# stevesuyao/KinectDepthMapEnhancement

Hardware: AMD Instinct MI355X
Metric: Mpixels/sec joint-bilateral filtered (640x480 & 1080p); % HBM roofline (higher is better)
Workload: dtype f32; 1 GPU; JointBilateralFilter::Process (K0 pre-smooth 5/30/30 + K1) on 64 x 640x480 synthetic RGB-D frames (64 per GPU), window 11 (radius 5), sigma_s 3 px, sigma_r 7.65/255, sigma_d 20 mm; frames_per_gpu=64, width=640, height=480, window=11, kernel_variant=auto (w11-pk2-16x16-false-v4)

## Files before the change

### kinectdepthmapenhancement_amd/csrc/jbf_fast.hip

```cpp
#include "kde_internal.h"
#include "kde_device_math.h"

#include <type_traits>

namespace kde {
namespace {

constexpr uint32_t kMagic = 0x4B000000u;
constexpr uint32_t kOff = 1u << 18;
constexpr uint32_t kInvalidBias = 0xFF000000u;
constexpr float kBiasF = 8388608.0f + 262144.0f;
constexpr uint32_t kNegHBits = 0xCB7C0000u;
constexpr double kScaleLog2 = 24.0;

struct FastArgs {
    const float* depth;
    const uint8_t* guide;
    float* out;
    int width, height, n;
    int tiles_x, tiles_y;
    FastDiv24 div_tiles, div_tx;
    float kc;
    float sd;
    float t_skip;
    float t2_skip;
    int cd_skip;
    int vec4;
    KDE_STAGE(float* stage_avg; unsigned* stage_counters; int stage_force;)
    const float* tab_dev;
    __attribute__((aligned(8))) float tab[882];
};

__device__ __forceinline__ uint32_t dot4(uint32_t a, uint32_t b, uint32_t c)
{
    return __builtin_amdgcn_udot4(a, b, c, false);
}


template <int WIN, int PX, int BX, int BY, bool CACHE, bool CSKIP>
__global__ __launch_bounds__(BX* BY) void jbf_fast_kernel(const FastArgs a)
{
    constexpr int R = WIN / 2;
    constexpr int NT = BX * BY;
    constexpr int TW = BX * PX, TH = BY;
    constexpr int LW = TW + 2 * R, LH = TH + 2 * R;
    constexpr int P = LW;
    constexpr int SEG = PX + 2 * R;
    __shared__ float s_d[LH * P];
    __shared__ uint32_t s_c[LH * P];
    __shared__ uint32_t s_n[LH * P];

    const unsigned nblk = gridDim.x;
    const unsigned lin = blockIdx.x;
    const unsigned per = nblk / 8, rem = nblk % 8;
    const unsigned xcd = lin % 8, slot = lin / 8;
    const unsigned id = xcd * per + (xcd < rem ? xcd : rem) + slot;
    const unsigned tiles = (unsigned)a.tiles_x * a.tiles_y;
    const unsigned frame_i = fastdiv24(id, a.div_tiles);
    const unsigned tile = id - frame_i * tiles;
    const int tyi = (int)fastdiv24(tile, a.div_tx), txi = tile - tyi * a.tiles_x;
    const int x0 = txi * TW, y0 = tyi * TH;

    const size_t frame = (size_t)frame_i * a.width * a.height;
    const float* __restrict__ depth = a.depth + frame;
    const uint8_t* __restrict__ guide = a.guide + frame * 3;
    const int tid = threadIdx.x;

    for (int i = tid; i < LW * LH; i += NT) {
        const int ly = i / LW, lx = i - ly * LW;
        const int gx = x0 + lx - R, gy = y0 + ly - R;
        float d = 0.0f;
        uint32_t c = 0;
        if (gx >= 0 && gx < a.width && gy >= 0 && gy < a.height) {
            const size_t q = (size_t)gy * a.width + gx;
            d = depth[q];
            const uint8_t* p = guide + q * 3;
            c = (uint32_t)p[0] | ((uint32_t)p[1] << 8) | ((uint32_t)p[2] << 16);
        }
        const bool valid = d > 50.0f;
        s_d[ly * P + lx] = valid ? d : 0.0f;
        s_c[ly * P + lx] = c;
        s_n[ly * P + lx] = valid ? (kMagic + kOff) - dot4(c, c, 0) : kInvalidBias;
    }
    __syncthreads();

    const int tx = tid % BX, ty = tid / BX;
    const int xb = x0 + tx * PX, y = y0 + ty;
    if (xb >= a.width || y >= a.height) return;

    uint32_t cc[PX];
    float cA[PX], skipA[PX];
    uint32_t thrU[PX];
#pragma unroll
    for (int k = 0; k < PX; k++) {
        cc[k] = s_c[(ty + R) * P + tx * PX + R + k];
        const uint32_t na = dot4(cc[k], cc[k], 0);
        cA[k] = -a.kc * (kBiasF + (float)na);
        skipA[k] = __builtin_fmaf(kBiasF + (float)na, a.kc, cA[k]);
        thrU[k] = CSKIP ? (kMagic + kOff) + na - (uint32_t)a.cd_skip : 0;
    }

    float arg[CACHE ? WIN * WIN * PX : 1];
    float wsum[PX], wgt[PX];
#pragma unroll
    for (int k = 0; k < PX; k++) wsum[k] = wgt[k] = 0.0f;

    auto arg1_of = [&](uint32_t cq, uint32_t nq, int k, float ls) -> float {
        const uint32_t u = (dot4(cq, cc[k], 0) << 1) + nq;
        float a1 = __builtin_fmaf(__uint_as_float(u), a.kc, cA[k]);
        if (CSKIP) a1 = (u <= thrU[k]) ? skipA[k] : a1;
        return a1 + ls;
    };

    auto pass1_row = [&](int i) {
        float dr[SEG];
        uint32_t cr[SEG], nr[SEG];
        const int rb = (ty + i) * P + tx * PX;
#pragma unroll
        for (int q = 0; q < SEG; q++) {
            dr[q] = s_d[rb + q];
            cr[q] = s_c[rb + q];
            nr[q] = s_n[rb + q];
        }
#pragma unroll
        for (int j = 0; j < WIN; j++) {
            const float ls = a.tab[i * WIN + j];
#pragma unroll
            for (int k = 0; k < PX; k++) {
                const float a1 = arg1_of(cr[j + k], nr[j + k], k, ls);
                if (CACHE) arg[(i * WIN + j) * PX + k] = a1;
                const float f = __builtin_amdgcn_exp2f(a1);
                wsum[k] = __builtin_fmaf(dr[j + k], f, wsum[k]);
                wgt[k] += f;
            }
        }
    };
    if (CACHE) {
#pragma unroll
        for (int i = 0; i < WIN; i++) pass1_row(i);
    } else {
#pragma unroll 1
        for (int i = 0; i < WIN; i++) pass1_row(i);
    }

    float c2[PX], num[PX], den[PX];
#pragma unroll
    for (int k = 0; k < PX; k++) {
        c2[k] = wsum[k] / wgt[k];
        num[k] = den[k] = 0.0f;
    }

    auto pass2_row = [&](int i) {
        float dr[SEG];
        uint32_t cr[SEG], nr[SEG];
        const int rb = (ty + i) * P + tx * PX;
#pragma unroll
        for (int q = 0; q < SEG; q++) {
            dr[q] = s_d[rb + q];
            if (!CACHE) {
                cr[q] = s_c[rb + q];
                nr[q] = s_n[rb + q];
            }
        }
#pragma unroll
        for (int j = 0; j < WIN; j++) {
            const float ls = CACHE ? 0.0f : a.tab[i * WIN + j];
#pragma unroll
            for (int k = 0; k < PX; k++) {
                const float a1 = CACHE ? arg[(i * WIN + j) * PX + k] : arg1_of(cr[j + k], nr[j + k], k, ls);
                const float t = (dr[j + k] - c2[k]) * a.sd;
                float a2 = __builtin_fmaf(-t, t, a1);
                a2 = (__builtin_fabsf(t) >= a.t_skip) ? a1 : a2;
                const float f = __builtin_amdgcn_exp2f(a2);
                num[k] = __builtin_fmaf(dr[j + k], f, num[k]);
                den[k] += f;
            }
        }
    };
    if (CACHE) {
#pragma unroll
        for (int i = 0; i < WIN; i++) pass2_row(i);
    } else {
#pragma unroll 1
        for (int i = 0; i < WIN; i++) pass2_row(i);
    }

    float* __restrict__ o = a.out + frame + (size_t)y * a.width + xb;
#pragma unroll
    for (int k = 0; k < PX; k++) {
        float r = 0.0f;
        if (wgt[k] > 0.0f) r = (den[k] == 0.0f) ? 0.0f : num[k] / den[k];
        if (xb + k < a.width) o[k] = r;
        KDE_STAGE(if (a.stage_avg && xb + k < a.width) a.stage_avg[frame + (size_t)y * a.width + xb + k] = c2[k];)
    }
}


typedef float f2 __attribute__((ext_vector_type(2)));
typedef uint32_t u2 __attribute__((ext_vector_type(2)));

__device__ __forceinline__ f2 pk_fma(f2 a, f2 b, f2 c) { return __builtin_elementwise_fma(a, b, c); }
__device__ __forceinline__ f2 bcast(float v) { return f2{v, v}; }
__device__ __forceinline__ f2 pk_add_clamp(f2 a, f2 b)
{
    f2 r;
    asm("v_pk_add_f32 %0, %1, %2 clamp" : "=v"(r) : "v"(a), "v"(b));
    return r;
}
__device__ __forceinline__ f2 pk_mul_clamp(f2 a, f2 b)
{
    f2 r;
    asm("v_pk_mul_f32 %0, %1, %2 clamp" : "=v"(r) : "v"(a), "v"(b));
    return r;
}

typedef unsigned short us2 __attribute__((ext_vector_type(2)));
__device__ __forceinline__ uint32_t pk_min_u16(uint32_t a, uint32_t b)
{
    return __builtin_bit_cast(uint32_t, __builtin_elementwise_min(__builtin_bit_cast(us2, a), __builtin_bit_cast(us2, b)));
}
__device__ __forceinline__ uint32_t pk_max_u16(uint32_t a, uint32_t b)
{
    return __builtin_bit_cast(uint32_t, __builtin_elementwise_max(__builtin_bit_cast(us2, a), __builtin_bit_cast(us2, b)));
}
template <int CTRL, int ROWS = 0xf>
__device__ __forceinline__ uint32_t dpp_mov(uint32_t v)
{
    return (uint32_t)__builtin_amdgcn_update_dpp((int)v, (int)v, CTRL, ROWS, 0xf, false);
}
template <class Op>
__device__ __forceinline__ uint32_t wave_reduce(uint32_t v, Op op)
{
    v = op(v, dpp_mov<0xb1>(v));
    v = op(v, dpp_mov<0x4e>(v));
    v = op(v, dpp_mov<0x124>(v));
    v = op(v, dpp_mov<0x128>(v));
    v = op(v, dpp_mov<0x142, 0xa>(v));
    v = op(v, dpp_mov<0x143, 0xc>(v));
    return (uint32_t)__builtin_amdgcn_readlane((int)v, 63);
}

constexpr int pk_min_waves(int win, int np, bool cache, bool cskip, bool elide_on)
{
    if (win >= 23) return 3;
    if (win == 5 && np == 1 && cache) return 5;
    if (np == 1 && !cskip && elide_on && !cache && win >= 9 && win <= 15) return win == 9 ? 8 : win == 11 ? 6 : 5;
    return 1;
}

template <int WIN, int NP, int BX, int BY, bool CACHE, bool CSKIP, bool VL, bool ELIDE_ON = true, int WTX = BX>
__global__ __launch_bounds__(BX* BY) __attribute__((amdgpu_waves_per_eu(pk_min_waves(WIN, NP, CACHE, CSKIP, ELIDE_ON))))
void jbf_pk_kernel(const FastArgs a)
{
    constexpr int CR = CACHE ? WIN : 0;
    constexpr int R = WIN / 2;
    constexpr int PX = 2 * NP;
    constexpr int NT = BX * BY;
    constexpr int WTY = 64 / WTX, WAVES_X = BX / WTX;
    static_assert(NT % 64 == 0 && 64 % WTX == 0 && BX % WTX == 0 && BY % WTY == 0, "whole wavefronts, each a WTX x WTY block of threads");
    constexpr int TW = BX * PX, TH = BY;
    constexpr int LH = TH + 2 * R;
    constexpr int S1 = 0;
    constexpr int RA = !VL ? R : ((R + 3) / 4 * 4);
    constexpr int SH = VL ? ((RA - R) & 1) : 0;
    constexpr bool ALIGNED = ((RA - R + SH) % 2) == 0;
    constexpr int G = (RA + TW + R + 3) / 4;
    constexpr int P = VL ? (SH + 4 * G + 1) / 2 * 2 : (TW + 2 * R);
    constexpr int SEGP = NP + R;
    constexpr int HALF = (WIN - 1) / 2;
    static_assert(RA >= R && P % 2 == 0 && (!VL || ((RA + S1) % 4 == 0 && TW % 4 == 0 && (SH != 0 || P % 4 == 0))), "tile geometry");
    __shared__ __attribute__((aligned(16))) float s_d[LH * P];
    __shared__ __attribute__((aligned(16))) uint32_t s_c[LH * P];
    __shared__ __attribute__((aligned(16))) float s_n[LH * P];

    const unsigned nblk = gridDim.x;
    const unsigned lin = blockIdx.x;
    const unsigned per = nblk / 8, rem = nblk % 8;
    const unsigned xcd = lin % 8, slot = lin / 8;
    const unsigned id = xcd * per + (xcd < rem ? xcd : rem) + slot;
    const unsigned tiles = (unsigned)a.tiles_x * a.tiles_y;
    const unsigned frame_i = fastdiv24(id, a.div_tiles);
    const unsigned tile = id - frame_i * tiles;
    const int tyi = (int)fastdiv24(tile, a.div_tx), txi = tile - tyi * a.tiles_x;
    const int x0 = txi * TW - S1, y0 = tyi * TH;
    const int o = x0 - RA;

    const size_t frame = (size_t)frame_i * a.width * a.height;
    const float* __restrict__ depth = a.depth + frame;
    const uint8_t* __restrict__ guide = a.guide + frame * 3;
    const int tid = threadIdx.x;

    constexpr bool ELIDE = WIN >= 9 && ELIDE_ON;

    if (!VL) {
        for (int i = tid; i < P * LH; i += NT) {
            const int ly = i / P, lx = i - ly * P;
            const int gx = o + lx, gy = y0 - R + ly;
            float d = 0.0f;
            uint32_t c = 0;
            const bool inside = gx >= 0 && gx < a.width && gy >= 0 && gy < a.height;
            if (inside) {
                const size_t q = (size_t)gy * a.width + gx;
                d = depth[q];
                const uint8_t* p = guide + q * 3;
                c = (uint32_t)p[0] | ((uint32_t)p[1] << 8) | ((uint32_t)p[2] << 16);
            }
            const bool valid = d > 50.0f;
            s_d[i] = valid ? d : 0.0f;
            s_c[i] = c;
            s_n[i] = __uint_as_float(dot4(c, c, kNegHBits));
        }
    }
    for (int g = tid; VL && g < G * LH; g += NT) {
        const int ly = g / G, gi = g - ly * G;
        const int gx = o + 4 * gi, gy = y0 - R + ly;
        float d[4] = {0.0f, 0.0f, 0.0f, 0.0f};
        uint32_t c[4] = {0u, 0u, 0u, 0u};
        if (gy >= 0 && gy < a.height) {
            const size_t q = (size_t)gy * a.width + gx;
            if (a.vec4 && gx >= 0 && gx + 3 < a.width) {
                const float4 dv = *reinterpret_cast<const float4*>(depth + q);
                const uint32_t* cp = reinterpret_cast<const uint32_t*>(guide + q * 3);
                const uint32_t w0 = cp[0], w1 = cp[1], w2 = cp[2];
                d[0] = dv.x; d[1] = dv.y; d[2] = dv.z; d[3] = dv.w;
                c[0] = w0 & 0xffffffu;
                c[1] = (w0 >> 24) | ((w1 & 0xffffu) << 8);
                c[2] = (w1 >> 16) | ((w2 & 0xffu) << 16);
                c[3] = w2 >> 8;
            } else {
#pragma unroll
                for (int k = 0; k < 4; k++) {
                    if (gx + k >= 0 && gx + k < a.width) {
                        d[k] = depth[q + k];
                        const uint8_t* p = guide + (q + k) * 3;
                        c[k] = (uint32_t)p[0] | ((uint32_t)p[1] << 8) | ((uint32_t)p[2] << 16);
                    }
                }
            }
        }
        float nn[4];
#pragma unroll
        for (int k = 0; k < 4; k++) {
            const bool valid = d[k] > 50.0f;
            d[k] = valid ? d[k] : 0.0f;
            nn[k] = __uint_as_float(dot4(c[k], c[k], kNegHBits));
        }
        const int li = ly * P + 4 * gi + SH;
        if constexpr (SH == 0) {
            *reinterpret_cast<float4*>(&s_d[li]) = make_float4(d[0], d[1], d[2], d[3]);
            *reinterpret_cast<uint4*>(&s_c[li]) = make_uint4(c[0], c[1], c[2], c[3]);
            *reinterpret_cast<float4*>(&s_n[li]) = make_float4(nn[0], nn[1], nn[2], nn[3]);
        } else {
#pragma unroll
            for (int k = 0; k < 4; k++) {
                s_d[li + k] = d[k];
                s_c[li + k] = c[k];
                s_n[li + k] = nn[k];
            }
        }
    }
    __syncthreads();

    const int wave = __builtin_amdgcn_readfirstlane(tid >> 6), lane = tid & 63;
    const int tx0 = WTX * (wave % WAVES_X), ty0 = WTY * (wave / WAVES_X);
    const int tx = tx0 + lane % WTX, ty = ty0 + lane / WTX;
    if (x0 + tx0 * PX >= a.width || y0 + ty0 >= a.height) return;

    bool tile_c = CSKIP, tile_d = true;
    if constexpr (ELIDE) {
        constexpr int RWP = (WTX * PX + 2 * R) / 2, RH = WTY + 2 * R;
        constexpr int NE = RWP * RH;
        const int sxw = SH + RA - R + tx0 * PX;
        const int gx0 = x0 + tx0 * PX - R, gy0 = y0 + ty0 - R;
        uint32_t dmin = 0xffffffffu, dmax = 0u;
        uint32_t brmin = 0x00ff00ffu, brmax = 0u, ggmin = 0x00ff00ffu, ggmax = 0u;
        auto scan = [&](auto masked_tag) {
            constexpr bool MASKED = decltype(masked_tag)::value;
            constexpr int QY = 64 / RWP, QP = 64 % RWP;
            int ry = lane / RWP, rp = lane - ry * RWP;
            int li = (ty0 + ry) * P + sxw + 2 * rp;
#pragma unroll
            for (int k = 0; k < (NE + 63) / 64; k++) {
                if (k > 0) {
                    const bool wrap = rp + QP >= RWP;
                    rp += wrap ? QP - RWP : QP;
                    ry += wrap ? QY + 1 : QY;
                    li += wrap ? (QY + 1) * P + 2 * (QP - RWP) : QY * P + 2 * QP;
                }
                if (64 * k + 63 < NE || lane + 64 * k < NE) {
                    const u2 d = *reinterpret_cast<const u2*>(&s_d[li]);
                    dmin = min(dmin, min(d.x - 1u, d.y - 1u));
                    dmax = max(dmax, max(d.x, d.y));
                    if constexpr (CSKIP) {
                        const u2 c = *reinterpret_cast<const u2*>(&s_c[li]);
                        uint32_t lo0 = c.x, lo1 = c.y, hi0 = c.x, hi1 = c.y;
                        if constexpr (MASKED) {
                            const bool iny = (unsigned)(gy0 + ry) < (unsigned)a.height;
                            const bool in0 = iny & ((unsigned)(gx0 + 2 * rp) < (unsigned)a.width);
                            const bool in1 = iny & ((unsigned)(gx0 + 2 * rp + 1) < (unsigned)a.width);
                            lo0 = in0 ? lo0 : 0x00ffffffu;
                            lo1 = in1 ? lo1 : 0x00ffffffu;
                            hi0 = in0 ? hi0 : 0u;
                            hi1 = in1 ? hi1 : 0u;
                        }
                        brmin = pk_min_u16(pk_min_u16(brmin, lo0 & 0x00ff00ffu), lo1 & 0x00ff00ffu);
                        brmax = pk_max_u16(pk_max_u16(brmax, hi0 & 0x00ff00ffu), hi1 & 0x00ff00ffu);
                        ggmin = pk_min_u16(ggmin, __builtin_amdgcn_perm(lo1, lo0, 0x0c050c01u));
                        ggmax = pk_max_u16(ggmax, __builtin_amdgcn_perm(hi1, hi0, 0x0c050c01u));
                    }
                }
            }
        };
        if (!CSKIP || (gx0 >= 0 && gx0 + 2 * RWP <= a.width && gy0 >= 0 && gy0 + RH <= a.height)) scan(std::false_type{});
        else scan(std::true_type{});
        const uint32_t w_dmin = wave_reduce(dmin, [](uint32_t p, uint32_t q) { return min(p, q); }) + 1u;
        const uint32_t w_dmax = wave_reduce(dmax, [](uint32_t p, uint32_t q) { return max(p, q); });
        if constexpr (CSKIP) {
            const uint32_t w_brmin = wave_reduce(brmin, pk_min_u16), w_brmax = wave_reduce(brmax, pk_max_u16);
            const uint32_t w_ggmin = wave_reduce(ggmin, pk_min_u16), w_ggmax = wave_reduce(ggmax, pk_max_u16);
            const int bmin = w_brmin & 0xffffu, bmax = w_brmax & 0xffffu, rmin = w_brmin >> 16, rmax = w_brmax >> 16;
            const int gmin = min(w_ggmin & 0xffffu, w_ggmin >> 16), gmax = max(w_ggmax & 0xffffu, w_ggmax >> 16);
            const int rb = bmax - bmin, rg = gmax - gmin, rr = rmax - rmin;
            if (bmax >= bmin) tile_c = rb * rb + rg * rg + rr * rr >= a.cd_skip;
        }
        if (w_dmax == 0u) {
            tile_d = false;
        } else {
            const float range = __uint_as_float(w_dmax) - __uint_as_float(w_dmin);
            const float slack = __uint_as_float(w_dmax) * (float)(WIN * WIN + 8) * 0x1p-24f;
            tile_d = !((range * 1.0001f + slack) * a.sd < a.t_skip);
        }
    }
    KDE_STAGE(if (a.stage_force) { tile_c = CSKIP; tile_d = true; })
    KDE_STAGE(if (a.stage_counters && lane == 0) {
        int body;
        if constexpr (!ELIDE) body = (CSKIP ? 1 : 0) + 2;
        else if constexpr (WIN >= 15) body = ((CSKIP && tile_c) || tile_d) ? (CSKIP ? 1 : 0) + 2 : 0;
        else body = ((CSKIP && tile_c) ? 1 : 0) + (tile_d ? 2 : 0);
        atomicAdd(&a.stage_counters[body], 1u);
    })

    const int xb = x0 + tx * PX, y = y0 + ty;
    if (xb >= a.width || y >= a.height) return;
    const int sx = SH + RA - R + tx * PX;

    uint32_t cc[PX];
    f2 negC[NP];
#pragma unroll
    for (int pp = 0; pp < NP; pp++) {
#pragma unroll
        for (int h = 0; h < 2; h++) {
            const int k = 2 * pp + h;
            cc[k] = s_c[(ty + R) * P + sx + R + k];
            const uint32_t na = dot4(cc[k], cc[k], 0);
            negC[pp][h] = -((float)kOff + (float)na);
        }
    }

    f2 kc2 = bcast(a.kc);
    asm volatile("" : "+v"(kc2));
    f2 arg[CR > 0 ? CR * WIN * NP : 1];
    f2 wsum[NP], wgt[NP];
#pragma unroll
    for (int pp = 0; pp < NP; pp++) wsum[pp] = wgt[pp] = bcast(0.0f);

    const f2 Tc = bcast((float)a.cd_skip);
    const f2 T2 = bcast(a.t2_skip);
    const f2 kBig = bcast(0x1p100f);

    auto unit_arg = [&](auto cs_tag, const u2* cp, const f2* np, int pp, int i, int u) -> f2 {
        constexpr bool CS = decltype(cs_tag)::value;
        uint32_t c0, c1;
        f2 hq;
        if (u <= HALF) {
            c0 = cp[pp + u].x; c1 = cp[pp + u].y; hq = np[pp + u];
        } else if (u < WIN - 1) {
            const int m = pp + (u - HALF);
            c0 = cp[m].y; c1 = cp[m].x; hq = __builtin_shufflevector(np[m], np[m], 1, 0);
        } else {
            c0 = cp[pp].y; c1 = cp[pp + HALF].x; hq = bcast(0.0f);
        }
        const f2 ab = f2{__uint_as_float(dot4(c0, cc[2 * pp], kMagic)), __uint_as_float(dot4(c1, cc[2 * pp + 1], kMagic))};
        f2 w;
        if (u == WIN - 1) {
            float w0 = __builtin_fmaf(ab.x, 2.0f, np[pp].y), w1 = __builtin_fmaf(ab.y, 2.0f, np[pp + HALF].x);
            asm("" : "+v"(w0));
            asm("" : "+v"(w1));
            w = f2{w0, w1};
        } else {
            w = pk_fma(ab, bcast(2.0f), hq);
        }
        const f2 ncd = w + negC[pp];
        f2 lsj;
        if constexpr (WIN > 21) {
            typedef const f2 __attribute__((address_space(4)))* cf2p;
            lsj = *(cf2p)(uintptr_t)(a.tab_dev + (i * WIN + u) * 2);
        } else {
            lsj = *reinterpret_cast<const f2*>(&a.tab[(i * WIN + u) * 2]);
        }
        if (CS) return pk_fma(ncd, pk_add_clamp(ncd, Tc) * kc2, lsj);
        return pk_fma(ncd, kc2, lsj);
    };
    auto unit_depth = [&](const f2* dp, int pp, int u) -> f2 {
        if (u <= HALF) return dp[pp + u];
        if (u < WIN - 1) return __builtin_shufflevector(dp[pp + (u - HALF)], dp[pp + (u - HALF)], 1, 0);
        return f2{dp[pp].y, dp[pp + HALF].x};
    };

    auto pass1_row = [&](auto cs_tag, auto keep_tag, int i) {
        constexpr bool KEEP = decltype(keep_tag)::value;
        f2 dp[SEGP], vp[SEGP];
        u2 cp[SEGP];
        f2 np[SEGP];
        const int rb = (ty + i) * P + sx;
#pragma unroll
        for (int m = 0; m < SEGP; m++) {
            dp[m] = ALIGNED ? *reinterpret_cast<const f2*>(&s_d[rb + 2 * m]) : f2{s_d[rb + 2 * m], s_d[rb + 2 * m + 1]};
            cp[m] = ALIGNED ? *reinterpret_cast<const u2*>(&s_c[rb + 2 * m]) : u2{s_c[rb + 2 * m], s_c[rb + 2 * m + 1]};
            np[m] = ALIGNED ? *reinterpret_cast<const f2*>(&s_n[rb + 2 * m]) : f2{s_n[rb + 2 * m], s_n[rb + 2 * m + 1]};
            vp[m] = pk_add_clamp(dp[m], dp[m]);
        }
#pragma unroll
        for (int pp = 0; pp < NP; pp++) {
#pragma unroll
            for (int u = 0; u < WIN; u++) {
                const f2 a1 = unit_arg(cs_tag, cp, np, pp, i, u);
                if constexpr (KEEP) arg[(i * NP + pp) * WIN + u] = a1;
                const f2 f = f2{__builtin_amdgcn_exp2f(a1.x), __builtin_amdgcn_exp2f(a1.y)};
                wsum[pp] = pk_fma(unit_depth(dp, pp, u), f, wsum[pp]);
                wgt[pp] = pk_fma(unit_depth(vp, pp, u), f, wgt[pp]);
            }
        }
    };
    f2 c2[NP], num[NP], den[NP];

    auto pass2_row = [&](auto cs_tag, auto ds_tag, auto keep_tag, int i) {
        constexpr bool DS = decltype(ds_tag)::value;
        constexpr bool KEEP = decltype(keep_tag)::value;
        f2 dp[SEGP], vp[SEGP];
        u2 cp[SEGP];
        f2 np[SEGP];
        const int rb = (ty + i) * P + sx;
#pragma unroll
        for (int m = 0; m < SEGP; m++) {
            dp[m] = ALIGNED ? *reinterpret_cast<const f2*>(&s_d[rb + 2 * m]) : f2{s_d[rb + 2 * m], s_d[rb + 2 * m + 1]};
            vp[m] = pk_add_clamp(dp[m], dp[m]);
            if constexpr (!KEEP) {
                cp[m] = ALIGNED ? *reinterpret_cast<const u2*>(&s_c[rb + 2 * m]) : u2{s_c[rb + 2 * m], s_c[rb + 2 * m + 1]};
                np[m] = ALIGNED ? *reinterpret_cast<const f2*>(&s_n[rb + 2 * m]) : f2{s_n[rb + 2 * m], s_n[rb + 2 * m + 1]};
            }
        }
#pragma unroll
        for (int pp = 0; pp < NP; pp++) {
#pragma unroll
            for (int u = 0; u < WIN; u++) {
                f2 a1;
                if constexpr (KEEP) a1 = arg[(i * NP + pp) * WIN + u];
                else a1 = unit_arg(cs_tag, cp, np, pp, i, u);
                const f2 dq = unit_depth(dp, pp, u);
                const f2 t = (dq - c2[pp]) * bcast(a.sd);
                f2 a2;
                if (DS) {
                    const f2 m = pk_mul_clamp(pk_fma(-t, t, T2), kBig);
                    a2 = pk_fma(-(t * m), t, a1);
                } else {
                    a2 = pk_fma(-t, t, a1);
                }
                const f2 f = f2{__builtin_amdgcn_exp2f(a2.x), __builtin_amdgcn_exp2f(a2.y)};
                num[pp] = pk_fma(dq, f, num[pp]);
                den[pp] = pk_fma(unit_depth(vp, pp, u), f, den[pp]);
            }
        }
    };
    auto run = [&](auto cs_tag, auto ds_tag) {
#pragma unroll
        for (int i = 0; i < CR; i++) pass1_row(cs_tag, std::true_type{}, i);
#pragma unroll 1
        for (int i = CR; i < WIN; i++) pass1_row(cs_tag, std::false_type{}, i);
#pragma unroll
        for (int pp = 0; pp < NP; pp++) {
            c2[pp] = wsum[pp] * f2{__builtin_amdgcn_rcpf(wgt[pp].x), __builtin_amdgcn_rcpf(wgt[pp].y)};
            num[pp] = den[pp] = bcast(0.0f);
        }
#pragma unroll
        for (int i = 0; i < CR; i++) pass2_row(cs_tag, ds_tag, std::true_type{}, i);
#pragma unroll 1
        for (int i = CR; i < WIN; i++) pass2_row(cs_tag, ds_tag, std::false_type{}, i);
    };
    using T_ = std::true_type;
    using F_ = std::false_type;
    if constexpr (!ELIDE) {
        run(std::integral_constant<bool, CSKIP>{}, T_{});
    } else if constexpr (WIN >= 15) {
        if ((CSKIP && tile_c) || tile_d) run(std::integral_constant<bool, CSKIP>{}, T_{});
        else run(F_{}, F_{});
    } else {
        if (!CSKIP || !tile_c) {
            if (tile_d) run(F_{}, T_{});
            else run(F_{}, F_{});
        } else {
            if (tile_d) run(T_{}, T_{});
            else run(T_{}, F_{});
        }
    }

    float* __restrict__ op = a.out + frame + (size_t)y * a.width + xb;
#pragma unroll
    for (int pp = 0; pp < NP; pp++) {
        float r0 = 0.0f, r1 = 0.0f;
        if (wgt[pp].x > 0.0f) r0 = (den[pp].x == 0.0f) ? 0.0f : num[pp].x * __builtin_amdgcn_rcpf(den[pp].x);
        if (wgt[pp].y > 0.0f) r1 = (den[pp].y == 0.0f) ? 0.0f : num[pp].y * __builtin_amdgcn_rcpf(den[pp].y);
        if (xb + 2 * pp >= 0 && xb + 2 * pp < a.width) op[2 * pp] = r0;
        if (xb + 2 * pp + 1 < a.width) op[2 * pp + 1] = r1;
        KDE_STAGE(if (a.stage_avg) {
            float* sp = a.stage_avg + frame + (size_t)y * a.width + xb;
            if (xb + 2 * pp >= 0 && xb + 2 * pp < a.width) sp[2 * pp] = c2[pp].x;
            if (xb + 2 * pp + 1 < a.width) sp[2 * pp + 1] = c2[pp].y;
        })
    }
}

template <int WIN, int NP, int BX, int BY, bool CACHE, bool VL, bool ELIDE_ON = true, int WTX = BX>
int launch_pk_variant(const JbfLaunch& l, const FastArgs& fa, bool cskip, hipStream_t s)
{
    FastArgs a = fa;
    a.tiles_x = ceil_div(l.width, BX * NP * 2);
    a.tiles_y = ceil_div(l.height, BY);
    const long long blocks = (long long)a.tiles_x * a.tiles_y * l.n;
    a.div_tiles = make_fastdiv24((uint32_t)(a.tiles_x * a.tiles_y), (uint64_t)blocks);
    a.div_tx = make_fastdiv24((uint32_t)a.tiles_x, (uint64_t)a.tiles_x * a.tiles_y);
    if (blocks > 0x7fffffffLL) return fail(KDE_ERR_INVALID, "jbf: batch too large for one launch");
    if (cskip)
        hipLaunchKernelGGL((jbf_pk_kernel<WIN, NP, BX, BY, CACHE, true, VL, ELIDE_ON, WTX>), dim3((unsigned)blocks), dim3(BX * BY), 0, s, a);
    else
        hipLaunchKernelGGL((jbf_pk_kernel<WIN, NP, BX, BY, CACHE, false, VL, ELIDE_ON, WTX>), dim3((unsigned)blocks), dim3(BX * BY), 0, s, a);
    KDE_HIP_TRY(hipGetLastError());
    return KDE_OK;
}

template <int WIN, int PX, int BX, int BY, bool CACHE>
int launch_variant(const JbfLaunch& l, const FastArgs& fa, bool cskip, hipStream_t s)
{
    FastArgs a = fa;
    a.tiles_x = ceil_div(l.width, BX * PX);
    a.tiles_y = ceil_div(l.height, BY);
    const long long blocks = (long long)a.tiles_x * a.tiles_y * l.n;
    a.div_tiles = make_fastdiv24((uint32_t)(a.tiles_x * a.tiles_y), (uint64_t)blocks);
    a.div_tx = make_fastdiv24((uint32_t)a.tiles_x, (uint64_t)a.tiles_x * a.tiles_y);
    if (blocks > 0x7fffffffLL) return fail(KDE_ERR_INVALID, "jbf: batch too large for one launch");
    if (cskip)
        hipLaunchKernelGGL((jbf_fast_kernel<WIN, PX, BX, BY, CACHE, true>), dim3((unsigned)blocks), dim3(BX * BY), 0, s, a);
    else
        hipLaunchKernelGGL((jbf_fast_kernel<WIN, PX, BX, BY, CACHE, false>), dim3((unsigned)blocks), dim3(BX * BY), 0, s, a);
    KDE_HIP_TRY(hipGetLastError());
    return KDE_OK;
}

struct Variant {
    const char* name;
    int window;
    bool packed;
    int (*launch)(const JbfLaunch&, const FastArgs&, bool, hipStream_t);
};

#define V(WIN, PX, BX, BY, CACHE) \
    {"w" #WIN "-sc" #PX "-" #BX "x" #BY "-" #CACHE, WIN, false, &launch_variant<WIN, PX, BX, BY, CACHE>}
#define K(WIN, NP, BX, BY, CACHE) \
    {"w" #WIN "-pk" #NP "-" #BX "x" #BY "-" #CACHE "-v4", WIN, true, &launch_pk_variant<WIN, NP, BX, BY, CACHE, true>}
#define KS(WIN, NP, BX, BY, CACHE) \
    {"w" #WIN "-pk" #NP "-" #BX "x" #BY "-" #CACHE "-v1", WIN, true, &launch_pk_variant<WIN, NP, BX, BY, CACHE, false>}
#define KN(WIN, NP, BX, BY, CACHE) \
    {"w" #WIN "-pk" #NP "-" #BX "x" #BY "-" #CACHE "-v4-noelide", WIN, true, &launch_pk_variant<WIN, NP, BX, BY, CACHE, true, false>}
#define KQ(WIN, NP, BX, BY, CACHE) \
    {"w" #WIN "-pk" #NP "-" #BX "x" #BY "-" #CACHE "-v4", WIN, true, &launch_pk_variant<WIN, NP, BX, BY, CACHE, true, true, 8>}
#define KR(WIN, NP, BX, BY, CACHE) \
    {"w" #WIN "-pk" #NP "-" #BX "x" #BY "-" #CACHE "-v4-rows", WIN, true, &launch_pk_variant<WIN, NP, BX, BY, CACHE, true>}
const Variant kVariants[] = {
    K(5, 1, 16, 16, true),  K(5, 1, 32, 8, true),   KS(5, 1, 16, 16, true),  K(5, 2, 32, 8, true),  K(5, 1, 32, 8, false),
    V(5, 2, 32, 8, true),   V(5, 1, 64, 4, true),
    K(7, 1, 16, 16, true),  K(7, 1, 32, 8, true),   KS(7, 1, 32, 8, true),  K(7, 1, 32, 8, false),  V(7, 1, 64, 4, true),
    KQ(11, 2, 16, 16, false), KR(11, 2, 16, 16, false), K(11, 2, 8, 32, false),
    KS(11, 2, 16, 16, false), KS(11, 1, 16, 16, false), K(11, 1, 16, 16, false), K(11, 1, 32, 8, false),
    KS(11, 1, 32, 8, false), KS(11, 2, 32, 8, false), V(11, 2, 16, 16, false), V(11, 1, 32, 8, false),
    KN(11, 2, 16, 16, false),
    K(19, 1, 16, 16, false), KS(19, 1, 16, 16, false), KS(19, 2, 16, 16, false), K(19, 2, 16, 16, false), K(19, 1, 32, 8, false),
    KS(19, 1, 32, 8, false), KS(19, 2, 32, 8, false), V(19, 2, 16, 16, false), V(19, 1, 32, 8, false),
    KN(19, 1, 16, 16, false),
    K(3, 1, 16, 16, true),   K(3, 2, 16, 16, true),
    K(9, 2, 16, 16, false),  K(9, 1, 16, 16, false),  KN(9, 2, 16, 16, false),
    K(13, 2, 16, 16, false), K(13, 1, 16, 16, false),
    K(15, 1, 16, 16, false), K(15, 2, 16, 16, false),
    K(17, 1, 16, 16, false), K(17, 2, 16, 16, false),
    K(21, 1, 16, 16, false), K(21, 2, 16, 16, false),
    K(23, 1, 16, 16, false), K(25, 1, 16, 16, false), K(27, 1, 16, 16, false), K(29, 1, 16, 16, false), K(31, 1, 16, 16, false),
};
static_assert(sizeof(FastArgs) <= 4096, "FastArgs is passed by value as the kernel-argument block");
#undef V
#undef K
#undef KS
#undef KN
#undef KQ
#undef KR
constexpr int kNumVariants = sizeof(kVariants) / sizeof(kVariants[0]);

}

int jbf_fast_variant_count() { return kNumVariants; }
const char* jbf_fast_variant_name(int v) { return (v >= 0 && v < kNumVariants) ? kVariants[v].name : "?"; }
int jbf_fast_variant_window(int v) { return (v >= 0 && v < kNumVariants) ? kVariants[v].window : 0; }

int jbf_fast_default_variant(const JbfLaunch& l)
{
    for (int v = 0; v < kNumVariants; v++)
        if (kVariants[v].window == l.window) return v;
    return -1;
}

bool jbf_fast_supported(const JbfLaunch& l)
{
    if (l.color_sigma == 0.0f || l.depth_sigma == 0.0f) return false;
    const double kc = 1.4426950408889634 / (double)l.color_den;
    if (!(kc * 1.0e38 > 1.0e4) || !(kc < 1.0e30)) return false;
    return jbf_fast_default_variant(l) >= 0;
}

void jbf_fast_fill_table(int W, const float* table_host, bool packed, float* out)
{
    const int HALF = (W - 1) / 2;
    auto lg = [&](int i, int j) {
        const float sv = table_host[i * W + j];
        return (float)(((sv == 0.0f) ? 0.0 : std::log2((double)sv)) + kScaleLog2);
    };
    if (!packed) {
        for (int i = 0; i < W; i++)
            for (int j = 0; j < W; j++) out[i * W + j] = lg(i, j);
        return;
    }
    for (int i = 0; i < W; i++)
        for (int u = 0; u < W; u++) {
            const int j0 = u <= HALF ? 2 * u : (u < W - 1 ? 2 * (u - HALF) + 1 : 1);
            const int j1 = u <= HALF ? 2 * u : (u < W - 1 ? 2 * (u - HALF) - 1 : W - 2);
            out[(i * W + u) * 2] = lg(i, j0);
            out[(i * W + u) * 2 + 1] = lg(i, j1);
        }
}

bool jbf_fast_needs_device_table(int window) { return window > 21; }

int launch_jbf_fast(const JbfLaunch& l, int variant, const float* table_host, hipStream_t s)
{
    if (variant < 0 || variant >= kNumVariants || kVariants[variant].window != l.window)
        return fail(KDE_ERR_INVALID, "jbf: variant %d does not implement window %d", variant, l.window);
    FastArgs a;
    memset(&a, 0, sizeof(a));
    a.depth = l.depth;
    a.guide = l.guide;
    a.out = l.out;
    a.width = l.width;
    a.height = l.height;
    a.n = l.n;
    const double log2e = 1.4426950408889634;
    a.kc = (float)(log2e / (double)l.color_den);
    a.sd = (float)std::sqrt(log2e / (double)l.depth_den);
    a.t_skip = std::isinf(l.d2_skip) ? INFINITY : (float)(std::sqrt((double)l.d2_skip) * std::sqrt(log2e / (double)l.depth_den));
    a.t2_skip = std::isinf(a.t_skip) ? 3.0e38f : a.t_skip * a.t_skip;
    a.cd_skip = l.cd_skip;
    a.vec4 = (l.width % 4 == 0) && ((reinterpret_cast<uintptr_t>(l.depth) & 15u) == 0) &&
             ((reinterpret_cast<uintptr_t>(l.guide) & 3u) == 0);
    KDE_STAGE(a.stage_avg = g_stage.jbf_avg; a.stage_counters = g_stage.counters; a.stage_force = g_stage.force_full_rules;)
    if (jbf_fast_needs_device_table(l.window)) {
        if (!l.log2_pk_dev) return fail(KDE_ERR_INVALID, "jbf: window %d needs the handle's device copy of the log2 table", l.window);
        a.tab_dev = l.log2_pk_dev;
    } else {
        jbf_fast_fill_table(l.window, table_host, kVariants[variant].packed, a.tab);
    }
    const bool cskip = l.cd_skip <= 195075;
    return kVariants[variant].launch(l, a, cskip, s);
}

}
```

Before: 17880 Mpixels/s.

## Encode invalid depth taps in the norm term and interleave LDS rows

For eligible template configurations, invalid depth samples get a huge negative norm value, which drives their exp2 weight to zero. The per-tap validity multiply then becomes a plain add in pass1 and pass2 when no color-skip tag applies. Shared arrays are also laid out row-interleaved (depth, color, norm rows adjacent) in a new s_rows buffer. This trims VALU work and registers in the inner loops, but the static shared declarations now allocate both layouts, which may raise LDS use and lower occupancy. The supported-kc check is tightened so the marker stays valid.

```diff
diff --git a/kinectdepthmapenhancement_amd/csrc/jbf_fast.hip b/kinectdepthmapenhancement_amd/csrc/jbf_fast.hip
--- a/kinectdepthmapenhancement_amd/csrc/jbf_fast.hip
+++ b/kinectdepthmapenhancement_amd/csrc/jbf_fast.hip
@@ -11,6 +11,9 @@
 constexpr uint32_t kInvalidBias = 0xFF000000u;
 constexpr float kBiasF = 8388608.0f + 262144.0f;
 constexpr uint32_t kNegHBits = 0xCB7C0000u;
+constexpr uint32_t kInvalidHBits = 0xFE800000u;
+constexpr double kMinKc = 1.0e-34;
+static_assert(kMinKc * 0x1p126 > 8000.0, "the invalid-tap marker must drive exp2 to 0 for every kc served");
 constexpr double kScaleLog2 = 24.0;
 
 struct FastArgs {
@@ -240,6 +243,13 @@
     return (uint32_t)__builtin_amdgcn_readlane((int)v, 63);
 }
 
+constexpr bool pk_invalid_by_code(int win, int np, bool cache, bool cskip)
+{
+    if (cache || win > 21) return false;
+    if (!cskip && ((np == 2 && win >= 17) || (np == 1 && win == 9))) return false;
+    return true;
+}
+
 constexpr int pk_min_waves(int win, int np, bool cache, bool cskip, bool elide_on)
 {
     if (win >= 23) return 3;
@@ -269,9 +279,15 @@
     constexpr int SEGP = NP + R;
     constexpr int HALF = (WIN - 1) / 2;
     static_assert(RA >= R && P % 2 == 0 && (!VL || ((RA + S1) % 4 == 0 && TW % 4 == 0 && (SH != 0 || P % 4 == 0))), "tile geometry");
+    constexpr bool BYCODE = pk_invalid_by_code(WIN, NP, CACHE, CSKIP);
+    constexpr int RP = BYCODE ? 3 * P : P;
     __shared__ __attribute__((aligned(16))) float s_d[LH * P];
     __shared__ __attribute__((aligned(16))) uint32_t s_c[LH * P];
     __shared__ __attribute__((aligned(16))) float s_n[LH * P];
+    __shared__ __attribute__((aligned(16))) uint32_t s_rows[3 * LH * P];
+#define l_d(k) (*(BYCODE ? reinterpret_cast<float*>(s_rows) + (k) : s_d + (k)))
+#define l_c(k) (*(BYCODE ? s_rows + P + (k) : s_c + (k)))
+#define l_n(k) (*(BYCODE ? reinterpret_cast<float*>(s_rows) + 2 * P + (k) : s_n + (k)))
 
     const unsigned nblk = gridDim.x;
     const unsigned lin = blockIdx.x;
@@ -306,9 +322,10 @@
                 c = (uint32_t)p[0] | ((uint32_t)p[1] << 8) | ((uint32_t)p[2] << 16);
             }
             const bool valid = d > 50.0f;
-            s_d[i] = valid ? d : 0.0f;
-            s_c[i] = c;
-            s_n[i] = __uint_as_float(dot4(c, c, kNegHBits));
+            const int li = ly * RP + lx;
+            l_d(li) = valid ? d : 0.0f;
+            l_c(li) = c;
+            l_n(li) = __uint_as_float((!BYCODE || valid) ? dot4(c, c, kNegHBits) : kInvalidHBits);
         }
     }
     for (int g = tid; VL && g < G * LH; g += NT) {
@@ -343,19 +360,19 @@
         for (int k = 0; k < 4; k++) {
             const bool valid = d[k] > 50.0f;
             d[k] = valid ? d[k] : 0.0f;
-            nn[k] = __uint_as_float(dot4(c[k], c[k], kNegHBits));
-        }
-        const int li = ly * P + 4 * gi + SH;
+            nn[k] = __uint_as_float((!BYCODE || valid) ? dot4(c[k], c[k], kNegHBits) : kInvalidHBits);
+        }
+        const int li = ly * RP + 4 * gi + SH;
         if constexpr (SH == 0) {
-            *reinterpret_cast<float4*>(&s_d[li]) = make_float4(d[0], d[1], d[2], d[3]);
-            *reinterpret_cast<uint4*>(&s_c[li]) = make_uint4(c[0], c[1], c[2], c[3]);
-            *reinterpret_cast<float4*>(&s_n[li]) = make_float4(nn[0], nn[1], nn[2], nn[3]);
+            *reinterpret_cast<float4*>(&l_d(li)) = make_float4(d[0], d[1], d[2], d[3]);
+            *reinterpret_cast<uint4*>(&l_c(li)) = make_uint4(c[0], c[1], c[2], c[3]);
+            *reinterpret_cast<float4*>(&l_n(li)) = make_float4(nn[0], nn[1], nn[2], nn[3]);
         } else {
 #pragma unroll
             for (int k = 0; k < 4; k++) {
-                s_d[li + k] = d[k];
-                s_c[li + k] = c[k];
-                s_n[li + k] = nn[k];
+                l_d(li + k) = d[k];
+                l_c(li + k) = c[k];
+                l_n(li + k) = nn[k];
             }
         }
     }
@@ -378,21 +395,21 @@
             constexpr bool MASKED = decltype(masked_tag)::value;
             constexpr int QY = 64 / RWP, QP = 64 % RWP;
             int ry = lane / RWP, rp = lane - ry * RWP;
-            int li = (ty0 + ry) * P + sxw + 2 * rp;
+            int li = (ty0 + ry) * RP + sxw + 2 * rp;
 #pragma unroll
             for (int k = 0; k < (NE + 63) / 64; k++) {
                 if (k > 0) {
                     const bool wrap = rp + QP >= RWP;
                     rp += wrap ? QP - RWP : QP;
                     ry += wrap ? QY + 1 : QY;
-                    li += wrap ? (QY + 1) * P + 2 * (QP - RWP) : QY * P + 2 * QP;
+                    li += wrap ? (QY + 1) * RP + 2 * (QP - RWP) : QY * RP + 2 * QP;
                 }
                 if (64 * k + 63 < NE || lane + 64 * k < NE) {
-                    const u2 d = *reinterpret_cast<const u2*>(&s_d[li]);
+                    const u2 d = *reinterpret_cast<const u2*>(&l_d(li));
                     dmin = min(dmin, min(d.x - 1u, d.y - 1u));
                     dmax = max(dmax, max(d.x, d.y));
                     if constexpr (CSKIP) {
-                        const u2 c = *reinterpret_cast<const u2*>(&s_c[li]);
+                        const u2 c = *reinterpret_cast<const u2*>(&l_c(li));
                         uint32_t lo0 = c.x, lo1 = c.y, hi0 = c.x, hi1 = c.y;
                         if constexpr (MASKED) {
                             const bool iny = (unsigned)(gy0 + ry) < (unsigned)a.height;
@@ -451,7 +468,7 @@
 #pragma unroll
         for (int h = 0; h < 2; h++) {
             const int k = 2 * pp + h;
-            cc[k] = s_c[(ty + R) * P + sx + R + k];
+            cc[k] = l_c((ty + R) * RP + sx + R + k);
             const uint32_t na = dot4(cc[k], cc[k], 0);
             negC[pp][h] = -((float)kOff + (float)na);
         }
@@ -508,17 +525,18 @@
     };
 
     auto pass1_row = [&](auto cs_tag, auto keep_tag, int i) {
+        constexpr bool VP = decltype(cs_tag)::value || !BYCODE;
         constexpr bool KEEP = decltype(keep_tag)::value;
-        f2 dp[SEGP], vp[SEGP];
+        f2 dp[SEGP], vp[VP ? SEGP : 1];
         u2 cp[SEGP];
         f2 np[SEGP];
-        const int rb = (ty + i) * P + sx;
+        const int rb = (ty + i) * RP + sx;
 #pragma unroll
         for (int m = 0; m < SEGP; m++) {
-            dp[m] = ALIGNED ? *reinterpret_cast<const f2*>(&s_d[rb + 2 * m]) : f2{s_d[rb + 2 * m], s_d[rb + 2 * m + 1]};
-            cp[m] = ALIGNED ? *reinterpret_cast<const u2*>(&s_c[rb + 2 * m]) : u2{s_c[rb + 2 * m], s_c[rb + 2 * m + 1]};
-            np[m] = ALIGNED ? *reinterpret_cast<const f2*>(&s_n[rb + 2 * m]) : f2{s_n[rb + 2 * m], s_n[rb + 2 * m + 1]};
-            vp[m] = pk_add_clamp(dp[m], dp[m]);
+            dp[m] = ALIGNED ? *reinterpret_cast<const f2*>(&l_d(rb + 2 * m)) : f2{l_d(rb + 2 * m), l_d(rb + 2 * m + 1)};
+            cp[m] = ALIGNED ? *reinterpret_cast<const u2*>(&l_c(rb + 2 * m)) : u2{l_c(rb + 2 * m), l_c(rb + 2 * m + 1)};
+            np[m] = ALIGNED ? *reinterpret_cast<const f2*>(&l_n(rb + 2 * m)) : f2{l_n(rb + 2 * m), l_n(rb + 2 * m + 1)};
+            if constexpr (VP) vp[m] = pk_add_clamp(dp[m], dp[m]);
         }
 #pragma unroll
         for (int pp = 0; pp < NP; pp++) {
@@ -528,26 +546,28 @@
                 if constexpr (KEEP) arg[(i * NP + pp) * WIN + u] = a1;
                 const f2 f = f2{__builtin_amdgcn_exp2f(a1.x), __builtin_amdgcn_exp2f(a1.y)};
                 wsum[pp] = pk_fma(unit_depth(dp, pp, u), f, wsum[pp]);
-                wgt[pp] = pk_fma(unit_depth(vp, pp, u), f, wgt[pp]);
+                if constexpr (VP) wgt[pp] = pk_fma(unit_depth(vp, pp, u), f, wgt[pp]);
+                else wgt[pp] = wgt[pp] + f;
             }
         }
     };
     f2 c2[NP], num[NP], den[NP];
 
     auto pass2_row = [&](auto cs_tag, auto ds_tag, auto keep_tag, int i) {
+        constexpr bool VP = decltype(cs_tag)::value || !BYCODE;
         constexpr bool DS = decltype(ds_tag)::value;
         constexpr bool KEEP = decltype(keep_tag)::value;
-        f2 dp[SEGP], vp[SEGP];
+        f2 dp[SEGP], vp[VP ? SEGP : 1];
         u2 cp[SEGP];
         f2 np[SEGP];
-        const int rb = (ty + i) * P + sx;
+        const int rb = (ty + i) * RP + sx;
 #pragma unroll
         for (int m = 0; m < SEGP; m++) {
-            dp[m] = ALIGNED ? *reinterpret_cast<const f2*>(&s_d[rb + 2 * m]) : f2{s_d[rb + 2 * m], s_d[rb + 2 * m + 1]};
-            vp[m] = pk_add_clamp(dp[m], dp[m]);
+            dp[m] = ALIGNED ? *reinterpret_cast<const f2*>(&l_d(rb + 2 * m)) : f2{l_d(rb + 2 * m), l_d(rb + 2 * m + 1)};
+            if constexpr (VP) vp[m] = pk_add_clamp(dp[m], dp[m]);
             if constexpr (!KEEP) {
-                cp[m] = ALIGNED ? *reinterpret_cast<const u2*>(&s_c[rb + 2 * m]) : u2{s_c[rb + 2 * m], s_c[rb + 2 * m + 1]};
-                np[m] = ALIGNED ? *reinterpret_cast<const f2*>(&s_n[rb + 2 * m]) : f2{s_n[rb + 2 * m], s_n[rb + 2 * m + 1]};
+                cp[m] = ALIGNED ? *reinterpret_cast<const u2*>(&l_c(rb + 2 * m)) : u2{l_c(rb + 2 * m), l_c(rb + 2 * m + 1)};
+                np[m] = ALIGNED ? *reinterpret_cast<const f2*>(&l_n(rb + 2 * m)) : f2{l_n(rb + 2 * m), l_n(rb + 2 * m + 1)};
             }
         }
 #pragma unroll
@@ -568,7 +588,8 @@
                 }
                 const f2 f = f2{__builtin_amdgcn_exp2f(a2.x), __builtin_amdgcn_exp2f(a2.y)};
                 num[pp] = pk_fma(dq, f, num[pp]);
-                den[pp] = pk_fma(unit_depth(vp, pp, u), f, den[pp]);
+                if constexpr (VP) den[pp] = pk_fma(unit_depth(vp, pp, u), f, den[pp]);
+                else den[pp] = den[pp] + f;
             }
         }
     };
@@ -619,6 +640,10 @@
         })
     }
 }
+
+#undef l_d
+#undef l_c
+#undef l_n
 
 template <int WIN, int NP, int BX, int BY, bool CACHE, bool VL, bool ELIDE_ON = true, int WTX = BX>
 int launch_pk_variant(const JbfLaunch& l, const FastArgs& fa, bool cskip, hipStream_t s)
@@ -720,7 +745,7 @@
 {
     if (l.color_sigma == 0.0f || l.depth_sigma == 0.0f) return false;
     const double kc = 1.4426950408889634 / (double)l.color_den;
-    if (!(kc * 1.0e38 > 1.0e4) || !(kc < 1.0e30)) return false;
+    if (!(kc > kMinKc) || !(kc < 1.0e30)) return false;
     return jbf_fast_default_variant(l) >= 0;
 }
 
```

Measured after the change: 18180 Mpixels/s, median of 6. 1.7% higher.
